# GarciaLnk/LlamaRec

Measured on AMD Instinct MI355X. Metric: users/sec through retrieve+rerank, higher is better.
Workload: dtype bf16; 1 GPU; beauty two-stage: LRURec(V=12086, L=50, D=64, 2 blocks) top-50 with history mask -> Llama-2-7b (32 layers, bf16, random init) single prefill -> verbalizer over 20 candidates; batching=token budget 32768 per step (llamarec_amd/packing.py), rmsnorm_folded_into_gemm=False, llama_layers=32, parallelism=dp1, collective_backend=nccl

## Files before the change

llamarec_amd/csrc/api_llama.hip:

```cpp
#include <math.h>
#include <stdlib.h>
#include <string.h>

#include <vector>

#include "llama_kernels.h"

typedef unsigned short u16;

extern "C" int lr_llama_create_ex(const LrLlamaConfig* cfg, const LrLlamaArch* arch, const LrLlamaWeightsDesc* w,
                                  lr_llama_t** out) {
  if (!cfg || !w || !out || !w->layers) LR_FAIL(LR_EINVAL, "lr_llama_create: null argument");
  const LrLlamaArch llama_arch = {0, 0, 1.0f, {0, 0, 0, 0, 0}};
  if (!arch) arch = &llama_arch;
  if (arch->norm_style < 0 || arch->norm_style > 1 || arch->mlp_act < 0 || arch->mlp_act > 1 ||
      !(arch->embed_scale > 0.f) || arch->embed_scale != arch->embed_scale)
    LR_FAIL(LR_EINVAL, "lr_llama_create_ex: arch norm_style=%d mlp_act=%d embed_scale=%g", arch->norm_style, arch->mlp_act,
            (double)arch->embed_scale);
  for (int i = 0; i < 5; ++i)
    if (arch->reserved[i]) LR_FAIL(LR_EINVAL, "lr_llama_create_ex: arch reserved word %d is not zero", i);
  if (cfg->num_layers < 1 || cfg->num_heads < 1 || cfg->num_kv_heads < 1 || cfg->vocab_size < 1)
    LR_FAIL(LR_EINVAL, "lr_llama_create: bad config");
  if (cfg->hidden_size % 8 != 0 || cfg->intermediate_size % 16 != 0)
    LR_FAIL(LR_EUNSUPPORTED, "lr_llama_create: hidden_size %% 8 and intermediate_size %% 16 must be 0");
// ... 9 lines not shown
      LR_FAIL(LR_EINVAL, "lr_llama_create: layer %d has a null weight", i);
  }
  lr_llama* h = (lr_llama*)calloc(1, sizeof(lr_llama));
  if (!h) LR_FAIL(LR_EINVAL, "lr_llama_create: out of host memory");
  h->cfg = *cfg;
  h->arch = *arch;
  h->embed = w->embed;
  h->final_norm = w->final_norm;
  h->lm_head = w->lm_head;
  h->prune_last = 1;
  h->layers = (LrLlamaLayerWeights*)malloc(sizeof(LrLlamaLayerWeights) * cfg->num_layers);
  memcpy(h->layers, w->layers, sizeof(LrLlamaLayerWeights) * cfg->num_layers);
  LR_CHECK_HIP(hipGetDevice(&h->device));
  *out = h;
  return LR_OK;
}

extern "C" int lr_llama_create(const LrLlamaConfig* cfg, const LrLlamaWeightsDesc* w, lr_llama_t** out) {
  return lr_llama_create_ex(cfg, nullptr, w, out);
}

extern "C" int lr_llama_set_variants(lr_llama_t* h, int32_t gemm_variant, int32_t attention_variant) {
  if (!h || (gemm_variant != 0 && gemm_variant != 1 && gemm_variant != 4 && gemm_variant != 5 && gemm_variant != 6) ||
      attention_variant < 0 || attention_variant > 9)
    LR_FAIL(LR_EINVAL, "lr_llama_set_variants: gemm in {0, 1, 4, 5, 6}, attention in {0, 1, 2, 3, 4, 5, 6, 7, 8, 9}");
  h->gemm_variant = gemm_variant;
  h->attn_variant = attention_variant;
  return LR_OK;
}

extern "C" int lr_llama_set_rope_scaling(lr_llama_t* h, const LrRopeScaling* s) {
  if (!h) LR_FAIL(LR_EINVAL, "lr_llama_set_rope_scaling: null handle");
  LR_RUN(lr_check_rope_scaling(s, "lr_llama_set_rope_scaling"));
  if (s) h->rope_scaling = *s;
  else memset(&h->rope_scaling, 0, sizeof(h->rope_scaling));
  return LR_OK;
}

static bool finite_nonneg(float v) { return v >= 0.f && v < __builtin_inff(); }

extern "C" int lr_llama_set_gemma2(lr_llama_t* h, const LrGemma2Ext* e) {
  if (!h) LR_FAIL(LR_EINVAL, "lr_llama_set_gemma2: null handle");
  const int L = h->cfg.num_layers;
  const uint16_t **an = nullptr, **mn = nullptr;
  float scale = 0.f;
  if (e) {
    if (!finite_nonneg(e->attn_softcap) || !finite_nonneg(e->final_softcap) || !finite_nonneg(e->attn_scale))
      LR_FAIL(LR_EINVAL, "lr_llama_set_gemma2: attn_softcap=%g final_softcap=%g attn_scale=%g (finite and >= 0)",
// ... 629 lines not shown
  return lr_launch_rope_table(cs, max_positions, head_dim, theta, (hipStream_t)hip_stream,
                              reinterpret_cast<unsigned*>(cs + (size_t)max_positions * head_dim), s);
}

extern "C" int lr_attention_varlen(const uint16_t* qkv, uint16_t* out, const int32_t* cu_seqlens,
                                   const int32_t* cu_seqlens_host, int32_t B, int32_t num_heads,
                                   int32_t num_kv_heads, int32_t head_dim, int32_t variant, void* hip_stream) {
  if (!qkv || !out || !cu_seqlens || !cu_seqlens_host || B < 1) LR_FAIL(LR_EINVAL, "lr_attention_varlen: bad argument");
  if (int rc = lr_check_segments(cu_seqlens_host, B, "lr_attention_varlen")) return rc;
  LrAttnKernel kernel;
  if (int rc = lr_resolve_attention({.variant = variant, .hd = head_dim}, &kernel)) return rc;
  return lr_launch_attention({.qkv = qkv, .out = out, .cu = cu_seqlens, .cu_host = cu_seqlens_host, .S = B,
                              .n_tok = cu_seqlens_host[B], .nh = num_heads, .nkv = num_kv_heads, .hd = head_dim},
                             kernel, (hipStream_t)hip_stream);
}

static int check_prefix_request(const char* who, const int32_t* cu_host, int S, int prefix_len, int nh, int nkv, int hd,
                                int variant) {
  if (!cu_host || S < 1 || prefix_len < 0 || nh < 1 || nkv < 1) LR_FAIL(LR_EINVAL, "%s: bad argument", who);
  if (int rc = lr_check_segments(cu_host, S, who)) return rc;
  if (nh % nkv != 0) LR_FAIL(LR_EINVAL, "%s: num_heads %d not a multiple of num_kv_heads %d", who, nh, nkv);
  if (prefix_len > 0 && (S < 2 || cu_host[1] != prefix_len))
    LR_FAIL(LR_EINVAL, "%s: segment 0 has %d rows, the shared prefix %d (and a prompt must follow it)", who, cu_host[1], prefix_len);
  const bool ok = (hd == 128 && (variant == 0 || variant == 2)) || (hd == 64 && (variant == 0 || variant == 5)) ||
                  (hd == 96 && (variant == 0 || variant == 7 || variant == 8)) || (hd == 256 && (variant == 0 || variant == 4 || variant == 9));
  if (!ok)
    LR_FAIL(LR_EUNSUPPORTED, "%s: variant %d at head_dim %d (0 / 2 at 128, 0 / 5 at 64, 0 / 7 / 8 at 96, 0 / 4 / 9 at 256)", who, variant, hd);
  return LR_OK;
}

extern "C" int lr_attention_varlen_prefix(const uint16_t* qkv, uint16_t* out, const int32_t* seg_starts,
                                          const int32_t* seg_starts_host, int32_t S, int32_t prefix_len, int32_t num_heads,
                                          int32_t num_kv_heads, int32_t head_dim, int32_t variant, void* hip_stream) {
  if (!qkv || !out || !seg_starts) LR_FAIL(LR_EINVAL, "lr_attention_varlen_prefix: null pointer");
  LR_RUN(check_prefix_request("lr_attention_varlen_prefix", seg_starts_host, S, prefix_len, num_heads, num_kv_heads, head_dim,
                              variant));
  LrAttnKernel kernel;
  LR_RUN(lr_resolve_attention({.variant = variant, .hd = head_dim, .prefix_len = prefix_len, .prefill = true}, &kernel));
  return lr_launch_attention({.qkv = qkv, .out = out, .cu = seg_starts, .cu_host = seg_starts_host, .S = S,
                              .n_tok = seg_starts_host[S], .nh = num_heads, .nkv = num_kv_heads, .hd = head_dim,
                              .prefix_len = prefix_len}, kernel, (hipStream_t)hip_stream);
}

extern "C" int lr_attention_last_rows(const uint16_t* kv, const uint16_t* q_last, uint16_t* out_last, const int32_t* seg_starts,
                                      const int32_t* seg_starts_host, int32_t S, int32_t prefix_len, int32_t num_heads,
                                      int32_t num_kv_heads, int32_t head_dim, int32_t variant, void* hip_stream) {
  if (!kv || !q_last || !out_last || !seg_starts) LR_FAIL(LR_EINVAL, "lr_attention_last_rows: null pointer");
  LR_RUN(check_prefix_request("lr_attention_last_rows", seg_starts_host, S, prefix_len, num_heads, num_kv_heads, head_dim,
                              variant));
  return lr_launch_attention_last(kv, q_last, out_last, seg_starts, seg_starts_host, S, seg_starts_host[S], num_heads,
// ... 456 lines not shown
```

llamarec_amd/csrc/api_llama_train.hip:

```cpp
#include <stdint.h>
#include <stdlib.h>
#include <string.h>

#include "llama_train.h"

typedef unsigned short u16;

struct lr_llama_lora {
  lr_llama* base;
  LrLoraTrainConfig cfg;
  LrLlamaLayerWeightsT* layers_t;
  const u16* lm_head_t;
  float *params, *grads, *m, *v;
  size_t n_params, per_layer;
  u16* work;
  size_t work_per_layer;
  float* scratch;
  int* ctr;
  uint32_t pass;
  int qcols, kcols, vcols;
  uint32_t mods;
  hipStream_t side;
  hipEvent_t ev_fork, ev_join;
  int deterministic;
// ... 519 lines not shown
  if (m < 1) LR_FAIL(LR_EINVAL, "lr_llama_lora_loss_grad: no labelled rows (m=%d)", m);
  hipStream_t st = (hipStream_t)hip_stream;
  const LrLlamaConfig& c = h->base->cfg;
  int n, maxT;
  LR_RUN(validate_batch(h, cu_seqlens_host, B, &n, &maxT));
  if (m > n) LR_FAIL(LR_EINVAL, "lr_llama_lora_loss_grad: %d labelled rows for %d tokens", m, n);
  const LoraMods md = lora_mods(c, h->cfg.r, h->mods);
  const bool det = h->deterministic != 0;
  const LoraWs ws = carve(c, md, n, B, m, c.num_layers, true, (char*)workspace, h->cfg.r, det, h->base->q_norm != nullptr);
  if (ws.total > workspace_bytes)
    LR_FAIL(LR_EWORKSPACE, "lr_llama_lora_loss_grad: workspace needs %zu bytes for %d tokens, have %zu", ws.total, n,
            workspace_bytes);
  const int d = c.hidden_size, f = c.intermediate_size, nh = c.num_heads, nkv = c.num_kv_heads, hd = c.head_dim;
  const int qw = (nh + 2 * nkv) * hd, r = h->cfg.r;
  const float scaling = h->cfg.alpha / (float)r, drop_p = h->cfg.dropout;
  const float drop_scale = drop_p > 0.f ? 1.0f / (1.0f - drop_p) : 1.0f;
  const int gv = h->base->gemm_variant == 5 ? 0 : h->base->gemm_variant;
  const int tw = md.tw, L = c.num_layers;
  LrAttnKernel fwd_kernel;
  LR_RUN(lr_resolve_attention({.variant = h->base->attn_variant, .hd = hd, .want_lse = true, .lora = true}, &fwd_kernel));
  const int attn_bwd_variant = fwd_kernel == LR_ATTN_HD64    ? 6
                               : fwd_kernel == LR_ATTN_HD96  ? 8
                               : fwd_kernel == LR_ATTN_HD256 ? 9
                                                             : h->base->attn_variant;
  h->pass += 1;
  if (!accumulate) LR_CHECK_HIP(hipMemsetAsync(h->grads, 0, h->n_params * sizeof(float), st));
  float* const scal = det ? ws.det_loss : h->scratch;
  float* const dp = ws.det_part;
  LR_CHECK_HIP(hipMemsetAsync(scal, 0, 2 * sizeof(float), st));
  LR_RUN(prep_adapters(h, st));
  LR_RUN(forward(h, packed_ids, cu_seqlens, cu_seqlens_host, B, n, maxT, ws, true, drop_p, st));

  LR_RUN(lr_launch_gather_rows(ws.x_final, loss_rows, m, d, ws.xg, st));
  LR_RUN(lr_launch_rmsnorm(ws.xg, h->base->final_norm, ws.hn, m, d, c.rms_eps, nullptr, st));
  LR_RUN(lr_launch_gemm({.A = ws.hn, .B = h->base->lm_head, .C = ws.logits, .M = m, .N = c.vocab_size, .K = d, .variant = gv}, st));
  LR_RUN(lr_launch_ce_bf16(ws.logits, m, c.vocab_size, loss_targets, grad_scale / (float)m, scal, st, det));
  LR_RUN(lr_launch_finish_loss(scal, m, out, st, det));
  LR_RUN(lr_launch_gemm({.A = ws.logits, .B = h->lm_head_t, .C = ws.dhn, .M = m, .N = d, .K = c.vocab_size, .variant = gv}, st));
  LR_CHECK_HIP(hipMemsetAsync(ws.dx, 0, (size_t)n * d * 2, st));
  LR_RUN(lr_launch_rmsnorm_bwd(ws.dhn, ws.xg, h->base->final_norm, nullptr, ws.dx, m, d, c.rms_eps, loss_rows, nullptr,
                               nullptr, 0, 0, 0.f, st));

  for (int l = c.num_layers - 1; l >= 0; --l) {
    const LrLlamaLayerWeights& w = h->base->layers[l];
    const LrLlamaLayerWeightsT& wt = h->layers_t[l];
    const LoraLayerSave s = slot(ws, l);
// ... 378 lines not shown
```

llamarec_amd/csrc/llama_attn.hip:

```cpp
#include <stdlib.h>

#include <type_traits>

#include "llama_kernels.h"
#include "lr_attn_util.h"
#include "lr_profile.h"

typedef unsigned short u16;
typedef __bf16 bf16x8 __attribute__((ext_vector_type(8)));
typedef __bf16 bf16x4 __attribute__((ext_vector_type(4)));
typedef short short4v __attribute__((ext_vector_type(4)));
typedef float floatx4 __attribute__((ext_vector_type(4)));
typedef u16 u16x4 __attribute__((ext_vector_type(4)));
typedef u16 u16x8 __attribute__((ext_vector_type(8)));

__global__ __launch_bounds__(256) void attn_generic_kernel(const u16* qkv, u16* out, const int32_t* cu, int B,
                                                           int n_tok, int nh, int nkv, int hd,
                                                           const int32_t* q_rows, float* lse, float scale_arg, float cap,
                                                           int window) {
  __shared__ float qs[4][256];
  const int wave = threadIdx.x >> 6, lane = threadIdx.x & 63;
  const int item = blockIdx.x * 4 + wave;
  if (item >= n_tok * nh) return;
  const int orow = item / nh, h = item % nh;
// ... 72 lines not shown
__device__ unsigned long long g_attn_stamps[64 * 8];
#define FA_WG_TRACE 8192
#ifdef LR_EXPERIMENTS
__device__ unsigned long long g_attn_wg[FA_WG_TRACE * 8];
#else
__device__ unsigned long long g_attn_wg[8];
#endif
#define FA_RT(dst)                                                                \
  if (STAMP) {                                                                    \
    __builtin_amdgcn_sched_barrier(0);                                            \
    asm volatile("s_memrealtime %0\n\ts_waitcnt lgkmcnt(0)" : "=s"(dst)::"memory"); \
    __builtin_amdgcn_sched_barrier(0);                                            \
  }
#define FA_STAMP(slot)                                                         \
  if (STAMP) {                                                                 \
    unsigned long long t_;                                                     \
    __builtin_amdgcn_sched_barrier(0);                                         \
    asm volatile("s_memtime %0\n\ts_waitcnt lgkmcnt(0)" : "=s"(t_)::"memory"); \
    __builtin_amdgcn_sched_barrier(0);                                         \
    stamp_acc[(slot)] += t_ - t_prev;                                          \
    t_prev = t_;                                                               \
  }

template <bool STAMP, bool LASTQ = false>
__global__ __launch_bounds__(256, 2) void attn_mfma128_kernel(const u16* __restrict__ qkv, u16* out,
                                                              const int32_t* cu, int prefix_len, int nh, int nkv,
                                                              int max_qblocks, int n_pairs, float* lse,
                                                              const u16* __restrict__ q_rows_last = nullptr) {
  unsigned long long stamp_acc[8] = {0, 0, 0, 0, 0, 0, 0, 0}, t_prev = 0;
  unsigned long long rt_entry = 0, rt_pro = 0, rt_loop = 0, rt_exit = 0;
  FA_RT(rt_entry)
  if (STAMP) asm volatile("s_memtime %0\n\ts_waitcnt lgkmcnt(0)" : "=s"(t_prev)::"memory");
  extern __shared__ __attribute__((aligned(16))) char smem[];
  const int hd = 128;
  int seg, h, qb;
  if (LASTQ) {
    const int id = blockIdx.x, stream = id & 7, pl = id >> 3;
    const int pair = pl * 8 + stream;
    if (pair >= n_pairs) return;
    seg = __builtin_amdgcn_readfirstlane(pair / nh);
    h = __builtin_amdgcn_readfirstlane(pair - seg * nh);
    if (prefix_len > 0 && seg == 0) return;
    qb = 0;
  } else {
    const int id = blockIdx.x, stream = id & 7, j = id >> 3;
    const int ppx = (n_pairs + 7) >> 3;
    const int n_light = min(max_qblocks, 2), n_heavy = max_qblocks - n_light;
    int pl;
    if (j < ppx * n_heavy) {
      pl = j / n_heavy;
      qb = max_qblocks - 1 - j % n_heavy;
// ... 8 lines not shown
    h = __builtin_amdgcn_readfirstlane(pair - seg * nh);
    qb = __builtin_amdgcn_readfirstlane(qb);
  }
  const int tok0 = cu[seg];
  const int P = (prefix_len > 0 && seg > 0) ? prefix_len : 0;
  const int T = P + cu[seg + 1] - tok0;
  if (LASTQ) qb = (T - 1) / FA_QROWS;
  if (qb * FA_QROWS >= T || (qb + 1) * FA_QROWS <= P) return;
  const int tid = threadIdx.x, lane = tid & 63;
  const int wave = __builtin_amdgcn_readfirstlane(tid >> 6);
  const int quad = lane >> 4, li = lane & 15;
  const int kvh = __builtin_amdgcn_readfirstlane(h / (nh / nkv));
  const int stride = LASTQ ? 2 * nkv * hd : (nh + 2 * nkv) * hd;
  const int koff0 = LASTQ ? kvh * hd : (nh + kvh) * hd, voff0 = koff0 + nkv * hd;
  const int vtok0 = tok0 - P;
  const u16* kbase = qkv + (size_t)vtok0 * stride + koff0;
  const u16* vbase = qkv + (size_t)vtok0 * stride + voff0;
  const u16* pkbase = qkv + koff0;
  const u16* pvbase = qkv + voff0;
  const int prompt = prefix_len > 0 ? seg - 1 : seg;

  bf16x8 qf[2][4];
  int qabs[2];
#pragma unroll
  for (int qt = 0; qt < 2; ++qt) {
    qabs[qt] = LASTQ ? T - 1 : qb * FA_QROWS + wave * 32 + qt * 16 + li;
    const int qr = min(max(qabs[qt], P), T - 1);
    const u16* qp = LASTQ ? q_rows_last + (size_t)prompt * nh * hd + h * hd + quad * 8
                          : qkv + (size_t)(vtok0 + qr) * stride + h * hd + quad * 8;
#pragma unroll
    for (int ks = 0; ks < 4; ++ks) qf[qt][ks] = *reinterpret_cast<const bf16x8*>(qp + ks * 32);
  }

  floatx4 ot[2][8];
#pragma unroll
  for (int qt = 0; qt < 2; ++qt)
#pragma unroll
    for (int dt = 0; dt < 8; ++dt) ot[qt][dt] = floatx4{0.f, 0.f, 0.f, 0.f};
  float m_run[2] = {-__builtin_inff(), -__builtin_inff()};
  float mthr[2] = {-__builtin_inff(), -__builtin_inff()};
  floatx4 l_acc[2] = {floatx4{0.f, 0.f, 0.f, 0.f}, floatx4{0.f, 0.f, 0.f, 0.f}};
  bf16x8 ones_f;
#pragma unroll
  for (int i = 0; i < 8; ++i) ones_f[i] = (__bf16)1.0f;

  const int q_last = min(qb * FA_QROWS + FA_QROWS - 1, T - 1);
  const int kb_last = q_last / FA_KB;
  const int wave_q_last = LASTQ ? T - 1 : qb * FA_QROWS + wave * 32 + 31;
  const float sl2 = 0.08838834764831845f * 1.4426950408889634f;
// ... 35 lines not shown
  };

  typedef __attribute__((address_space(3))) char lds_char;
  lds_char* const lds = (lds_char*)smem;
  lds_char *kb_off[4], *vb_off[8];
#pragma unroll
  for (int ks = 0; ks < 4; ++ks) kb_off[ks] = lds + (li * 256 + (((ks * 4 + quad) ^ li) << 4));
  {
    const int qp = li >> 2, p4 = li & 3;
#pragma unroll
    for (int dt = 0; dt < 8; ++dt) vb_off[dt] = lds + (v_off(quad * 4 + qp, dt * 2 + (p4 >> 1)) + 8 * (p4 & 1));
  }

  stage(0, 0);
#pragma unroll
  for (int qt = 0; qt < 2; ++qt)
#pragma unroll
    for (int ks = 0; ks < 4; ++ks) asm volatile("" ::"v"(qf[qt][ks]));
  asm volatile("s_waitcnt vmcnt(0)" ::: "memory");
  __syncthreads();
  FA_STAMP(0)
  FA_RT(rt_pro)

  auto block = [&](const int kb, auto buf_c) {
    constexpr int BUF = decltype(buf_c)::value;
    constexpr int KS = BUF * FA_STAGE_BYTES, VS = KS + FA_TILE_BYTES;
    if (kb < kb_last) stage(kb + 1, BUF ^ 1);
    FA_STAMP(1)

    if (kb * FA_KB <= wave_q_last && wave_q_last >= P && (!LASTQ || wave == 0)) {
      floatx4 st[2][4];
#pragma unroll
      for (int qt = 0; qt < 2; ++qt)
#pragma unroll
        for (int nt = 0; nt < 4; ++nt) st[qt][nt] = floatx4{0.f, 0.f, 0.f, 0.f};
      typedef __attribute__((address_space(3))) const bf16x8 lds_bf16x8;
      bf16x8 kf[2][4];
#pragma unroll
      for (int nt = 0; nt < 4; ++nt) kf[0][nt] = *reinterpret_cast<lds_bf16x8*>(kb_off[0] + (KS + nt * 4096));
#pragma unroll
      for (int ks = 0; ks < 4; ++ks) {
        if (ks < 3) {
#pragma unroll
          for (int nt = 0; nt < 4; ++nt)
            kf[(ks + 1) & 1][nt] = *reinterpret_cast<lds_bf16x8*>(kb_off[ks + 1] + (KS + nt * 4096));
        }
#pragma unroll
        for (int nt = 0; nt < 4; ++nt)
#pragma unroll
          for (int qt = 0; qt < 2; ++qt)
            st[qt][nt] = __builtin_amdgcn_mfma_f32_16x16x32_bf16(kf[ks & 1][nt], qf[qt][ks], st[qt][nt], 0, 0, 0);
      }

      if (STAMP) asm volatile("" ::"v"(st[0][0]), "v"(st[1][3]));
      FA_STAMP(2)
      bf16x8 pa[2][2];
      const bool diag = (kb * FA_KB + FA_KB - 1) > (LASTQ ? T - 1 : qb * FA_QROWS + wave * 32);
#pragma unroll
      for (int qt = 0; qt < 2; ++qt) {
        float mx = -__builtin_inff();
        if (diag) {
#pragma unroll
          for (int nt = 0; nt < 4; ++nt)
#pragma unroll
            for (int r = 0; r < 4; ++r) {
              const int key = kb * FA_KB + nt * 16 + quad * 4 + r;
              st[qt][nt][r] = (key <= qabs[qt]) ? st[qt][nt][r] : -__builtin_inff();
            }
          __builtin_amdgcn_sched_barrier(0);
        }
        mx = fa_max3(st[qt][0][0], st[qt][0][1], st[qt][0][2]);
        mx = fa_max3(mx, st[qt][0][3], st[qt][1][0]);
#pragma unroll
        for (int nt = 1; nt < 4; ++nt) {
          mx = fa_max3(mx, st[qt][nt][1], st[qt][nt][2]);
          if (nt < 3) mx = fa_max3(mx, st[qt][nt][3], st[qt][nt + 1][0]);
        }
        mx = fa_max2(mx, st[qt][3][3]);
        if (__any(mx > mthr[qt])) {
          const float rmx = fa_max_xor16_32(mx);
          const bool grew = rmx > mthr[qt];
          const float m_new = grew ? rmx * sl2 : m_run[qt];
          const float alpha = __builtin_amdgcn_exp2f(m_run[qt] - m_new);
#pragma unroll
          for (int r = 0; r < 4; ++r) l_acc[qt][r] *= alpha;
#pragma unroll
          for (int dt = 0; dt < 8; ++dt)
#pragma unroll
            for (int r = 0; r < 4; ++r) ot[qt][dt][r] *= alpha;
          m_run[qt] = m_new;
          mthr[qt] = (m_new + FA_DEFER) * inv_sl2;
        }
        const float m_new = m_run[qt];
#pragma unroll
        for (int nt = 0; nt < 4; ++nt)
#pragma unroll
          for (int r = 0; r < 4; ++r) {
            const float p = __builtin_amdgcn_exp2f(__builtin_fmaf(st[qt][nt][r], sl2, -m_new));
            pa[qt][nt >> 1][(nt & 1) * 4 + r] = (__bf16)p;
          }
      }

      if (STAMP) asm volatile("" ::"v"(pa[0][0]), "v"(pa[1][1]));
      FA_STAMP(3)
#pragma unroll
      for (int ks2 = 0; ks2 < 2; ++ks2) {
#pragma unroll
        for (int qt = 0; qt < 2; ++qt) l_acc[qt] = __builtin_amdgcn_mfma_f32_16x16x32_bf16(ones_f, pa[qt][ks2], l_acc[qt], 0, 0, 0);
#pragma unroll
        for (int dt = 0; dt < 8; ++dt) {
          const short4v t0 = __builtin_amdgcn_ds_read_tr16_b64_v4i16(
              (__attribute__((address_space(3))) short4v*)(vb_off[dt] + (VS + ks2 * 8192)));
          const short4v t1 = __builtin_amdgcn_ds_read_tr16_b64_v4i16(
              (__attribute__((address_space(3))) short4v*)(vb_off[dt] + (VS + ks2 * 8192 + 4096)));
          bf16x8 vf;
          const bf16x4 b0 = __builtin_bit_cast(bf16x4, t0), b1 = __builtin_bit_cast(bf16x4, t1);
#pragma unroll
          for (int r = 0; r < 4; ++r) {
            vf[r] = b0[r];
            vf[4 + r] = b1[r];
          }
#pragma unroll
          for (int qt = 0; qt < 2; ++qt)
            ot[qt][dt] = __builtin_amdgcn_mfma_f32_16x16x32_bf16(vf, pa[qt][ks2], ot[qt][dt], 0, 0, 0);
        }
      }
    }
    if (STAMP) asm volatile("" ::"v"(ot[0][0]), "v"(ot[1][7]));
    FA_STAMP(4)
    asm volatile("s_waitcnt vmcnt(0)" ::: "memory");
    __syncthreads();
    FA_STAMP(5)
  };
  for (int kb = 0; kb <= kb_last; kb += 2) {
    block(kb, std::integral_constant<int, 0>{});
    if (kb + 1 <= kb_last) block(kb + 1, std::integral_constant<int, 1>{});
  }

  FA_RT(rt_loop)
#pragma unroll
  for (int qt = 0; qt < 2; ++qt) {
    const float l = l_acc[qt][0];
    const float inv = 1.0f / l;
    if (!LASTQ && qabs[qt] < T && qabs[qt] >= P && lse && quad == 0)
      lse[(size_t)(vtok0 + qabs[qt]) * nh + h] = (m_run[qt] + __builtin_amdgcn_logf(l)) * 0.6931471805599453f;
    const bool live = LASTQ ? (wave == 0 && qt == 0 && li == 0) : (qabs[qt] < T && qabs[qt] >= P);
    u16* op = out + (size_t)(LASTQ ? prompt : vtok0 + (live ? qabs[qt] : P)) * nh * hd + h * hd + (quad & 1) * 16 + (quad >> 1) * 8;
#pragma unroll
    for (int k = 0; k < 4; ++k) {
      unsigned a[2], b[2];
#pragma unroll
      for (int w = 0; w < 2; ++w) {
        a[w] = (unsigned)f2bf(ot[qt][2 * k][2 * w] * inv) | ((unsigned)f2bf(ot[qt][2 * k][2 * w + 1] * inv) << 16);
        b[w] = (unsigned)f2bf(ot[qt][2 * k + 1][2 * w] * inv) | ((unsigned)f2bf(ot[qt][2 * k + 1][2 * w + 1] * inv) << 16);
        const auto sw = __builtin_amdgcn_permlane16_swap(a[w], b[w], false, false);
        a[w] = sw[0];
        b[w] = sw[1];
      }
      if (live) {
// ... 32 lines not shown
extern "C" int lr_debug_attn_stamps(unsigned long long* out, int n) {
  if (!out || n < 1 || n > 64 * 8) LR_FAIL(LR_EINVAL, "lr_debug_attn_stamps: bad arguments");
  LR_CHECK_HIP(hipMemcpyFromSymbol(out, HIP_SYMBOL(g_attn_stamps), (size_t)n * sizeof(unsigned long long)));
  return LR_OK;
}
#endif

int lr_launch_attention_rows(const u16* qkv, u16* out, const int32_t* cu, int B, const int32_t* q_rows,
                             int n_rows, int nh, int nkv, int hd, hipStream_t st, float scale, float cap, int window) {
  if (n_rows <= 0) return LR_OK;
  if (window < 0) LR_FAIL(LR_EINVAL, "attention: window %d", window);
  if (hd > 256) LR_FAIL(LR_EUNSUPPORTED, "attention: head_dim %d > 256", hd);
  const int items = n_rows * nh;
  hipLaunchKernelGGL(attn_generic_kernel, dim3((items + 3) / 4), dim3(256), 0, st, qkv, out, cu, B, n_rows,
                     nh, nkv, hd, q_rows, (float*)nullptr, scale, cap, window);
  LR_CHECK_LAUNCH("attn_generic_kernel(rows)");
  return LR_OK;
}

int lr_resolve_attention(const LrAttnRequest& r, LrAttnKernel* kernel) {
  const int hd = r.hd;
  if (r.cap > 0.f) {
    if (r.want_lse) LR_FAIL(LR_EINVAL, "attention: no lse with a soft cap");
    if (r.variant == 2 || r.variant == 3 || r.variant == 5 || r.variant == 6 || ((r.variant == 7 || r.variant == 8) && hd == 96) ||
        (r.variant == 9 && hd == 256))
      LR_FAIL(LR_EUNSUPPORTED, "attention variant %d has no soft-capped form (0 / 4 at head_dim 256, 1 generic)", r.variant);
    if (r.variant != 0 && r.variant != 1 && r.variant != 4) LR_FAIL(LR_EINVAL, "attention: unknown variant %d", r.variant);
    if (r.variant != 1 && hd == 256 && r.cap <= LR_SOFTCAP_MFMA_MAX) {
      *kernel = LR_ATTN_HD256;
      return LR_OK;
    }
    if (r.prefix_len > 0) LR_FAIL(LR_EUNSUPPORTED, "attention: the generic kernel reads no shared prefix (soft cap, head_dim %d)", hd);
    *kernel = LR_ATTN_GENERIC;
    return LR_OK;
  }
  switch (r.variant) {
    case 0:
      if (hd == 128) *kernel = (r.have_items_ws && !r.prefill) ? LR_ATTN_ROWS256 : LR_ATTN_MFMA128;
      else if (hd == 256 && (r.prefill || r.lora || r.prefix_len > 0)) *kernel = LR_ATTN_HD256;
      else if (hd == 96 && (r.prefill || r.lora || r.prefix_len > 0)) *kernel = LR_ATTN_HD96;
      else *kernel = (hd == 64 && (r.prefill || r.lora || r.prefix_len > 0)) ? LR_ATTN_HD64 : LR_ATTN_GENERIC;
      if (r.prefix_len > 0 && *kernel == LR_ATTN_GENERIC)
        LR_FAIL(LR_EUNSUPPORTED, "attention: no kernel reads a shared prefix at head_dim %d", hd);
      if (r.prefix_len > 0 && r.want_lse && hd != 128)
        LR_FAIL(LR_EINVAL, "attention: no lse with a shared prefix at head_dim %d", hd);
      return LR_OK;
    case 1:
// ... 18 lines not shown
      if (hd != 64) LR_FAIL(LR_EUNSUPPORTED, "attention variant 5 needs head_dim 64 (got %d)", hd);
      *kernel = LR_ATTN_HD64;
      return LR_OK;
    case 6:
      if (hd != 64) LR_FAIL(LR_EUNSUPPORTED, "attention variant 6 needs head_dim 64 (got %d)", hd);
      if (r.want_lse && r.prefix_len > 0) LR_FAIL(LR_EINVAL, "attention variant 6 writes no lse with a shared prefix");
      *kernel = LR_ATTN_HD64;
      return LR_OK;
    case 7:
      if (r.want_lse) LR_FAIL(LR_EINVAL, "attention variant 7 (head_dim-96 MFMA) writes no lse");
      if (hd != 96) LR_FAIL(LR_EUNSUPPORTED, "attention variant 7 needs head_dim 96 (got %d)", hd);
      *kernel = LR_ATTN_HD96;
      return LR_OK;
    case 8:
      if (hd != 96) LR_FAIL(LR_EUNSUPPORTED, "attention variant 8 needs head_dim 96 (got %d)", hd);
      if (r.want_lse && r.prefix_len > 0) LR_FAIL(LR_EINVAL, "attention variant 8 writes no lse with a shared prefix");
      *kernel = LR_ATTN_HD96;
      return LR_OK;
    case 9:
      if (hd != 256) LR_FAIL(LR_EUNSUPPORTED, "attention variant 9 needs head_dim 256 (got %d)", hd);
      if (r.want_lse && r.prefix_len > 0) LR_FAIL(LR_EINVAL, "attention variant 9 writes no lse with a shared prefix");
      *kernel = LR_ATTN_HD256;
      return LR_OK;
  }
  LR_FAIL(LR_EINVAL, "attention: unknown variant %d (0 auto, 1 generic, 2 = head_dim-128 MFMA, 3 = 256-row tiles, "
          "4 = head_dim-256 MFMA, 5 = head_dim-64 MFMA, 6 = head_dim-64 MFMA for training, 7 = head_dim-96 MFMA, "
          "8 = head_dim-96 MFMA for training, 9 = head_dim-256 MFMA for training)", r.variant);
}

int lr_launch_attention(const LrAttnArgs& a, LrAttnKernel kernel, hipStream_t st) {
  const int32_t* cu_host = a.cu_host;
  const int B = a.S, n_tok = a.n_tok, nh = a.nh, nkv = a.nkv, hd = a.hd, prefix_len = a.prefix_len;
  if (n_tok <= 0 || B <= 0) return LR_OK;
  if (a.cap < 0.f || a.scale < 0.f || a.cap != a.cap || a.scale != a.scale)
    LR_FAIL(LR_EINVAL, "attention: scale %g cap %g", (double)a.scale, (double)a.cap);
  if (a.cap > 0.f && kernel != LR_ATTN_HD256 && kernel != LR_ATTN_GENERIC)
    LR_FAIL(LR_EUNSUPPORTED, "attention: kernel %d has no soft-capped form", (int)kernel);
  if (a.window < 0) LR_FAIL(LR_EINVAL, "attention: window %d", a.window);
  if (a.window > 0 && ((kernel != LR_ATTN_HD256 && kernel != LR_ATTN_GENERIC) || prefix_len != 0 || a.lse || a.cap > 0.f))
    LR_FAIL(LR_EUNSUPPORTED, "attention: a sliding window runs on the head_dim-256 MFMA kernel or the generic one, without a "
            "shared prefix, lse or a soft cap (kernel %d, prefix %d)", (int)kernel, prefix_len);
  if (kernel == LR_ATTN_ROWS256) return lr_launch_attention256(a, st);
  if (nh % nkv != 0) LR_FAIL(LR_EINVAL, "attention: num_heads %d not a multiple of num_kv_heads %d", nh, nkv);
  if (kernel == LR_ATTN_HD256) {
    if (prefix_len < 0 || (a.lse && (prefix_len > 0 || a.cap > 0.f)))
      LR_FAIL(LR_EINVAL, "attention: the head_dim-256 MFMA kernel writes no lse with a shared prefix or a soft cap (prefix %d)",
              prefix_len);
    if (a.cap > 0.f) return lr_launch_attention_hd256_softcap(a, st);
    if (a.window > 0) return lr_launch_attention_hd256_window(a, st);
    return prefix_len > 0 ? lr_launch_attention_hd256_prefix(a, st) : lr_launch_attention_hd256(a, st);
  }
  if (kernel == LR_ATTN_HD64) {
    if (prefix_len < 0) LR_FAIL(LR_EINVAL, "attention: shared prefix of %d tokens", prefix_len);
    return prefix_len > 0 ? lr_launch_attention_hd64_prefix(a, st) : lr_launch_attention_hd64(a, st);
  }
  if (kernel == LR_ATTN_HD96) {
    if (prefix_len < 0 || (prefix_len > 0 && a.lse))
      LR_FAIL(LR_EINVAL, "attention: the head_dim-96 MFMA kernel writes no lse with a shared prefix (prefix %d)", prefix_len);
    return prefix_len > 0 ? lr_launch_attention_hd96_prefix(a, st) : lr_launch_attention_hd96(a, st);
  }
  if (prefix_len < 0 || (prefix_len > 0 && (kernel != LR_ATTN_MFMA128 || cu_host[1] - cu_host[0] != prefix_len)))
    LR_FAIL(LR_EINVAL, "attention: shared prefix of %d tokens needs the head_dim-128 MFMA kernel and segment 0 = the prefix",
            prefix_len);
  const LrAttnPlan pl = lr_attn_plan(cu_host, B, prefix_len, nh, hd, FA_QROWS, nh);
  LrProfScope prof(kernel == LR_ATTN_MFMA128 ? LR_PROF_ATTN_MFMA : LR_PROF_ATTN_GENERIC, pl.work, st);
  if (kernel == LR_ATTN_MFMA128) {
    if (hd != 128) LR_FAIL(LR_EUNSUPPORTED, "attention variant 2 needs head_dim 128 (got %d)", hd);
    const int mq = pl.mq;
    if (mq == 0) return LR_OK;
    LR_RUN(lr_attn_check_grid(pl));
    if ((long long)n_tok * (nh + 2 * nkv) * hd * 2 > 0x7fffffffLL * 2)
      LR_FAIL(LR_EUNSUPPORTED, "attention: packed qkv of %d tokens exceeds the 4 GiB a buffer descriptor addresses", n_tok);
    const int n_pairs = (int)pl.n_pairs;
    const unsigned grid = (unsigned)pl.grid;
    static bool lds_set[LR_MAX_DEVICES] = {};
    if (int rc = lr_ensure_dynamic_lds(reinterpret_cast<const void*>(attn_mfma128_kernel<false>), 2 * FA_STAGE_BYTES, lds_set))
      return rc;
#ifdef LR_EXPERIMENTS
    static bool lds_set_stamp[LR_MAX_DEVICES] = {};
    const char* stamp_env = getenv("LR_ATTN_STAMPS");
    if (stamp_env && stamp_env[0] == '1') {
      const char* one_env = getenv("LR_ATTN_ONE_PER_CU");
      const int lds_bytes = (one_env && one_env[0] == '1') ? 104 * 1024 : 2 * FA_STAGE_BYTES;
      if (int rc = lr_ensure_dynamic_lds(reinterpret_cast<const void*>(attn_mfma128_kernel<true>), 104 * 1024, lds_set_stamp))
        return rc;
      hipLaunchKernelGGL(attn_mfma128_kernel<true>, dim3(grid), dim3(256), lds_bytes, st, a.qkv, a.out, a.cu,
                         prefix_len, nh, nkv, mq, n_pairs, a.lse);
    } else
#endif
      hipLaunchKernelGGL(attn_mfma128_kernel<false>, dim3(grid), dim3(256), 2 * FA_STAGE_BYTES, st, a.qkv, a.out, a.cu,
                         prefix_len, nh, nkv, mq, n_pairs, a.lse);
    LR_CHECK_LAUNCH("attn_mfma128_kernel");
  } else {
    if (hd > 256) LR_FAIL(LR_EUNSUPPORTED, "attention: head_dim %d > 256", hd);
    const int items = n_tok * nh;
    hipLaunchKernelGGL(attn_generic_kernel, dim3((items + 3) / 4), dim3(256), 0, st, a.qkv, a.out, a.cu, B,
                       n_tok, nh, nkv, hd, (const int32_t*)nullptr, a.lse, a.scale, a.cap, a.window);
// ... 41 lines not shown
```

llamarec_amd/csrc/llama_kernels.h:

```cpp
#ifndef LLAMA_KERNELS_H
#define LLAMA_KERNELS_H

#include "lr_common.h"
#include "lr_profile.h"

__device__ __forceinline__ float bf2f(unsigned short b) {
  return __builtin_bit_cast(float, (unsigned int)b << 16);
}
__device__ __forceinline__ unsigned short f2bf(float f) {
  return __builtin_bit_cast(unsigned short, (__bf16)f);
}
__device__ __forceinline__ unsigned short swiglu_bf16(float g, float u) {
  float s = bf2f(f2bf(g * __builtin_amdgcn_rcpf(1.0f + __expf(-g))));
  return f2bf(s * u);
}

__device__ __forceinline__ unsigned short geglu_bf16(float g, float u) {
  const float t = tanhf(0.7978845608028654f * (g + 0.044715f * g * g * g));
  float s = bf2f(f2bf(0.5f * g * (1.0f + t)));
  return f2bf(s * u);
}
template <int NS>
__device__ __forceinline__ unsigned short rms_apply(unsigned short w, unsigned short x, float rstd) {
  if (NS == 0) return f2bf(bf2f(w) * bf2f(f2bf(bf2f(x) * rstd)));
// ... 113 lines not shown
    const double P = (prefix_len > 0 && b > 0) ? prefix_len : 0, T = P + cu_host[b + 1] - cu_host[b];
    p.work += 4.0 * nh * hd * (T * (T + 1) / 2 - P * (P + 1) / 2);
    p.maxT = p.maxT > (int)T ? p.maxT : (int)T;
  }
  p.mq = (p.maxT + q_rows - 1) / q_rows;
  p.n_pairs = (long long)S * pairs_per_prompt;
  p.grid = 8 * ((p.n_pairs + 7) / 8) * p.mq;
  return p;
}
static inline LrAttnPlan lr_attn_plan_last(const int32_t* cu_host, int S, int prefix_len, int nh, int hd, int grid_multiple) {
  LrAttnPlan p;
  for (int b = (prefix_len > 0 ? 1 : 0); b < S; ++b)
    p.work += 4.0 * nh * hd * (double)((prefix_len > 0 ? prefix_len : 0) + cu_host[b + 1] - cu_host[b]);
  p.n_pairs = (long long)S * nh;
  p.grid = grid_multiple * ((p.n_pairs + grid_multiple - 1) / grid_multiple);
  return p;
}
static inline int lr_attn_check_grid(const LrAttnPlan& p) {
  if (p.grid > 0x7fffffffLL) LR_FAIL(LR_EUNSUPPORTED, "attention: %lld workgroups exceed the grid limit", p.grid);
  return LR_OK;
}

enum LrAttnKernel {
  LR_ATTN_GENERIC = 1, LR_ATTN_MFMA128 = 2, LR_ATTN_ROWS256 = 3, LR_ATTN_HD256 = 4, LR_ATTN_HD64 = 5, LR_ATTN_HD96 = 7
};

#define LR_SOFTCAP_MFMA_MAX 256.0f
static inline bool lr_attention_reads_prefix(int variant, int hd, float cap = 0.f) {
  if (cap > 0.f) return hd == 256 && (variant == 0 || variant == 4) && cap <= LR_SOFTCAP_MFMA_MAX;
  if (hd == 128) return variant != 1;
  if (hd == 64) return variant == 0 || variant == 5 || variant == 6;
  if (hd == 96) return variant == 0 || variant == 7 || variant == 8;
  if (hd == 256) return variant == 0 || variant == 4 || variant == 9;
  return false;
}
static inline bool lr_attention_has_last_row_mode(int kernel, int hd) {
  return (hd == 128 && kernel != 1 ) || kernel == 4  || kernel == 5  ||
         kernel == 7 ;
}
struct LrAttnRequest {
  int variant, hd, prefix_len = 0;
  bool want_lse = false, have_items_ws = false, prefill = false, lora = false;
  float cap = 0.f;
};
int lr_resolve_attention(const LrAttnRequest& r, LrAttnKernel* kernel);

struct LrAttnArgs {
// ... 112 lines not shown
```

Baseline: 159.2 users/s.

## Balance causal attention waves with mirrored row groups and per-group diagonal skipping

The default head_dim-128 MFMA attention kernel now gives each wave a mirrored pair of 16-row query groups (wave and 7-wave) instead of 32 contiguous rows. It runs full key blocks on a fast unmasked path and handles diagonal blocks per group, skipping MFMA tiles that lie fully above the causal diagonal. This is meant to even out causal work across waves and cut wasted score and PV compute on diagonal tiles. The old contiguous mapping stays reachable as a new variant 10. The cost is more code paths, extra register pressure and more branching.

```diff
diff --git a/llamarec_amd/csrc/api_llama.hip b/llamarec_amd/csrc/api_llama.hip
--- a/llamarec_amd/csrc/api_llama.hip
+++ b/llamarec_amd/csrc/api_llama.hip
@@ -55,8 +55,8 @@
 
 extern "C" int lr_llama_set_variants(lr_llama_t* h, int32_t gemm_variant, int32_t attention_variant) {
   if (!h || (gemm_variant != 0 && gemm_variant != 1 && gemm_variant != 4 && gemm_variant != 5 && gemm_variant != 6) ||
-      attention_variant < 0 || attention_variant > 9)
-    LR_FAIL(LR_EINVAL, "lr_llama_set_variants: gemm in {0, 1, 4, 5, 6}, attention in {0, 1, 2, 3, 4, 5, 6, 7, 8, 9}");
+      attention_variant < 0 || attention_variant > 10)
+    LR_FAIL(LR_EINVAL, "lr_llama_set_variants: gemm in {0, 1, 4, 5, 6}, attention in {0, 1, 2, 3, 4, 5, 6, 7, 8, 9, 10}");
   h->gemm_variant = gemm_variant;
   h->attn_variant = attention_variant;
   return LR_OK;
@@ -732,10 +732,10 @@
   if (nh % nkv != 0) LR_FAIL(LR_EINVAL, "%s: num_heads %d not a multiple of num_kv_heads %d", who, nh, nkv);
   if (prefix_len > 0 && (S < 2 || cu_host[1] != prefix_len))
     LR_FAIL(LR_EINVAL, "%s: segment 0 has %d rows, the shared prefix %d (and a prompt must follow it)", who, cu_host[1], prefix_len);
-  const bool ok = (hd == 128 && (variant == 0 || variant == 2)) || (hd == 64 && (variant == 0 || variant == 5)) ||
+  const bool ok = (hd == 128 && (variant == 0 || variant == 2 || variant == 10)) || (hd == 64 && (variant == 0 || variant == 5)) ||
                   (hd == 96 && (variant == 0 || variant == 7 || variant == 8)) || (hd == 256 && (variant == 0 || variant == 4 || variant == 9));
   if (!ok)
-    LR_FAIL(LR_EUNSUPPORTED, "%s: variant %d at head_dim %d (0 / 2 at 128, 0 / 5 at 64, 0 / 7 / 8 at 96, 0 / 4 / 9 at 256)", who, variant, hd);
+    LR_FAIL(LR_EUNSUPPORTED, "%s: variant %d at head_dim %d (0 / 2 / 10 at 128, 0 / 5 at 64, 0 / 7 / 8 at 96, 0 / 4 / 9 at 256)", who, variant, hd);
   return LR_OK;
 }
 
diff --git a/llamarec_amd/csrc/api_llama_train.hip b/llamarec_amd/csrc/api_llama_train.hip
--- a/llamarec_amd/csrc/api_llama_train.hip
+++ b/llamarec_amd/csrc/api_llama_train.hip
@@ -565,6 +565,7 @@
   const int attn_bwd_variant = fwd_kernel == LR_ATTN_HD64    ? 6
                                : fwd_kernel == LR_ATTN_HD96  ? 8
                                : fwd_kernel == LR_ATTN_HD256 ? 9
+                               : fwd_kernel == LR_ATTN_MFMA128_STRAIGHT ? 2
                                                              : h->base->attn_variant;
   h->pass += 1;
   if (!accumulate) LR_CHECK_HIP(hipMemsetAsync(h->grads, 0, h->n_params * sizeof(float), st));
diff --git a/llamarec_amd/csrc/llama_attn.hip b/llamarec_amd/csrc/llama_attn.hip
--- a/llamarec_amd/csrc/llama_attn.hip
+++ b/llamarec_amd/csrc/llama_attn.hip
@@ -118,11 +118,12 @@
     t_prev = t_;                                                               \
   }
 
-template <bool STAMP, bool LASTQ = false>
+template <bool STAMP, bool LASTQ = false, bool STRAIGHT = false>
 __global__ __launch_bounds__(256, 2) void attn_mfma128_kernel(const u16* __restrict__ qkv, u16* out,
                                                               const int32_t* cu, int prefix_len, int nh, int nkv,
                                                               int max_qblocks, int n_pairs, float* lse,
                                                               const u16* __restrict__ q_rows_last = nullptr) {
+  constexpr bool GROUPS = !LASTQ && !STRAIGHT;
   unsigned long long stamp_acc[8] = {0, 0, 0, 0, 0, 0, 0, 0}, t_prev = 0;
   unsigned long long rt_entry = 0, rt_pro = 0, rt_loop = 0, rt_exit = 0;
   FA_RT(rt_entry)
@@ -177,9 +178,15 @@
 
   bf16x8 qf[2][4];
   int qabs[2];
+  int g_need[2] = {-1, -1}, g_nv[2] = {4, 4};
 #pragma unroll
   for (int qt = 0; qt < 2; ++qt) {
-    qabs[qt] = LASTQ ? T - 1 : qb * FA_QROWS + wave * 32 + qt * 16 + li;
+    const int g0 = qb * FA_QROWS + (GROUPS ? (qt ? 7 - wave : wave) * 16 : wave * 32 + qt * 16);
+    if (GROUPS && g0 < T && g0 + 15 >= P) {
+      g_need[qt] = g0 / FA_KB;
+      g_nv[qt] = ((g0 & (FA_KB - 1)) >> 4) + 1;
+    }
+    qabs[qt] = LASTQ ? T - 1 : g0 + li;
     const int qr = min(max(qabs[qt], P), T - 1);
     const u16* qp = LASTQ ? q_rows_last + (size_t)prompt * nh * hd + h * hd + quad * 8
                           : qkv + (size_t)(vtok0 + qr) * stride + h * hd + quad * 8;
@@ -261,19 +268,24 @@
   FA_STAMP(0)
   FA_RT(rt_pro)
 
-  auto block = [&](const int kb, auto buf_c) {
+  auto block = [&](const int kb, auto buf_c, auto hot_c) {
     constexpr int BUF = decltype(buf_c)::value;
+    constexpr bool HOT = decltype(hot_c)::value;
     constexpr int KS = BUF * FA_STAGE_BYTES, VS = KS + FA_TILE_BYTES;
     if (kb < kb_last) stage(kb + 1, BUF ^ 1);
     FA_STAMP(1)
 
-    if (kb * FA_KB <= wave_q_last && wave_q_last >= P && (!LASTQ || wave == 0)) {
-      floatx4 st[2][4];
+    typedef __attribute__((address_space(3))) const bf16x8 lds_bf16x8;
+    typedef std::integral_constant<int, 0> c0;
+    typedef std::integral_constant<int, 1> c1;
+    typedef std::integral_constant<int, 3> c3;
+    typedef std::integral_constant<int, 4> c4;
+
+    auto scores_pair = [&](floatx4(&st)[2][4]) __attribute__((always_inline)) {
 #pragma unroll
       for (int qt = 0; qt < 2; ++qt)
 #pragma unroll
         for (int nt = 0; nt < 4; ++nt) st[qt][nt] = floatx4{0.f, 0.f, 0.f, 0.f};
-      typedef __attribute__((address_space(3))) const bf16x8 lds_bf16x8;
       bf16x8 kf[2][4];
 #pragma unroll
       for (int nt = 0; nt < 4; ++nt) kf[0][nt] = *reinterpret_cast<lds_bf16x8*>(kb_off[0] + (KS + nt * 4096));
@@ -290,80 +302,141 @@
           for (int qt = 0; qt < 2; ++qt)
             st[qt][nt] = __builtin_amdgcn_mfma_f32_16x16x32_bf16(kf[ks & 1][nt], qf[qt][ks], st[qt][nt], 0, 0, 0);
       }
-
-      if (STAMP) asm volatile("" ::"v"(st[0][0]), "v"(st[1][3]));
-      FA_STAMP(2)
-      bf16x8 pa[2][2];
-      const bool diag = (kb * FA_KB + FA_KB - 1) > (LASTQ ? T - 1 : qb * FA_QROWS + wave * 32);
-#pragma unroll
-      for (int qt = 0; qt < 2; ++qt) {
-        float mx = -__builtin_inff();
-        if (diag) {
-#pragma unroll
-          for (int nt = 0; nt < 4; ++nt)
-#pragma unroll
-            for (int r = 0; r < 4; ++r) {
-              const int key = kb * FA_KB + nt * 16 + quad * 4 + r;
-              st[qt][nt][r] = (key <= qabs[qt]) ? st[qt][nt][r] : -__builtin_inff();
-            }
-          __builtin_amdgcn_sched_barrier(0);
-        }
-        mx = fa_max3(st[qt][0][0], st[qt][0][1], st[qt][0][2]);
-        mx = fa_max3(mx, st[qt][0][3], st[qt][1][0]);
-#pragma unroll
-        for (int nt = 1; nt < 4; ++nt) {
-          mx = fa_max3(mx, st[qt][nt][1], st[qt][nt][2]);
-          if (nt < 3) mx = fa_max3(mx, st[qt][nt][3], st[qt][nt + 1][0]);
-        }
-        mx = fa_max2(mx, st[qt][3][3]);
-        if (__any(mx > mthr[qt])) {
-          const float rmx = fa_max_xor16_32(mx);
-          const bool grew = rmx > mthr[qt];
-          const float m_new = grew ? rmx * sl2 : m_run[qt];
-          const float alpha = __builtin_amdgcn_exp2f(m_run[qt] - m_new);
-#pragma unroll
-          for (int r = 0; r < 4; ++r) l_acc[qt][r] *= alpha;
-#pragma unroll
-          for (int dt = 0; dt < 8; ++dt)
-#pragma unroll
-            for (int r = 0; r < 4; ++r) ot[qt][dt][r] *= alpha;
-          m_run[qt] = m_new;
-          mthr[qt] = (m_new + FA_DEFER) * inv_sl2;
-        }
-        const float m_new = m_run[qt];
+    };
+
+    auto softmax_group = [&](auto qt_c, floatx4(&st)[2][4], bf16x8(&pa)[2][2], const bool masked, auto nv_c) __attribute__((always_inline)) {
+      constexpr int qt = decltype(qt_c)::value;
+      constexpr bool NV_RT = std::is_same<decltype(nv_c), int>::value;
+      const int nv = nv_c;
+      float mx;
+      if (masked) {
 #pragma unroll
         for (int nt = 0; nt < 4; ++nt)
+#pragma unroll
+          for (int r = 0; r < 4; ++r) {
+            const int key = kb * FA_KB + nt * 16 + quad * 4 + r;
+            st[qt][nt][r] = (key <= qabs[qt]) ? st[qt][nt][r] : -__builtin_inff();
+          }
+        __builtin_amdgcn_sched_barrier(0);
+      }
+      mx = fa_max3(st[qt][0][0], st[qt][0][1], st[qt][0][2]);
+      mx = fa_max3(mx, st[qt][0][3], st[qt][1][0]);
+#pragma unroll
+      for (int nt = 1; nt < 4; ++nt) {
+        mx = fa_max3(mx, st[qt][nt][1], st[qt][nt][2]);
+        if (nt < 3) mx = fa_max3(mx, st[qt][nt][3], st[qt][nt + 1][0]);
+      }
+      mx = fa_max2(mx, st[qt][3][3]);
+      if (__any(mx > mthr[qt])) {
+        const float rmx = fa_max_xor16_32(mx);
+        const bool grew = rmx > mthr[qt];
+        const float m_new = grew ? rmx * sl2 : m_run[qt];
+        const float alpha = __builtin_amdgcn_exp2f(m_run[qt] - m_new);
+#pragma unroll
+        for (int r = 0; r < 4; ++r) l_acc[qt][r] *= alpha;
+#pragma unroll
+        for (int dt = 0; dt < 8; ++dt)
+#pragma unroll
+          for (int r = 0; r < 4; ++r) ot[qt][dt][r] *= alpha;
+        m_run[qt] = m_new;
+        mthr[qt] = (m_new + FA_DEFER) * inv_sl2;
+      }
+      const float m_new = m_run[qt];
+#pragma unroll
+      for (int nt = 0; nt < 4; ++nt) {
+        if (nt < nv) {
+          if constexpr (NV_RT) asm volatile("");
 #pragma unroll
           for (int r = 0; r < 4; ++r) {
             const float p = __builtin_amdgcn_exp2f(__builtin_fmaf(st[qt][nt][r], sl2, -m_new));
             pa[qt][nt >> 1][(nt & 1) * 4 + r] = (__bf16)p;
           }
-      }
-
+        } else {
+#pragma unroll
+          for (int r = 0; r < 4; ++r) pa[qt][nt >> 1][(nt & 1) * 4 + r] = (__bf16)0.0f;
+        }
+      }
+    };
+
+    auto pv_step = [&](auto qm_c, auto ks2_c, bf16x8(&pa)[2][2]) __attribute__((always_inline)) {
+      constexpr int QM = decltype(qm_c)::value, ks2 = decltype(ks2_c)::value;
+#pragma unroll
+      for (int qt = 0; qt < 2; ++qt)
+        if ((QM >> qt) & 1) l_acc[qt] = __builtin_amdgcn_mfma_f32_16x16x32_bf16(ones_f, pa[qt][ks2], l_acc[qt], 0, 0, 0);
+#pragma unroll
+      for (int dt = 0; dt < 8; ++dt) {
+        const short4v t0 = __builtin_amdgcn_ds_read_tr16_b64_v4i16(
+            (__attribute__((address_space(3))) short4v*)(vb_off[dt] + (VS + ks2 * 8192)));
+        const short4v t1 = __builtin_amdgcn_ds_read_tr16_b64_v4i16(
+            (__attribute__((address_space(3))) short4v*)(vb_off[dt] + (VS + ks2 * 8192 + 4096)));
+        bf16x8 vf;
+        const bf16x4 b0 = __builtin_bit_cast(bf16x4, t0), b1 = __builtin_bit_cast(bf16x4, t1);
+#pragma unroll
+        for (int r = 0; r < 4; ++r) {
+          vf[r] = b0[r];
+          vf[4 + r] = b1[r];
+        }
+#pragma unroll
+        for (int qt = 0; qt < 2; ++qt)
+          if ((QM >> qt) & 1) ot[qt][dt] = __builtin_amdgcn_mfma_f32_16x16x32_bf16(vf, pa[qt][ks2], ot[qt][dt], 0, 0, 0);
+      }
+    };
+
+    auto both_groups = [&](const bool masked) __attribute__((always_inline)) {
+      floatx4 st[2][4];
+      bf16x8 pa[2][2];
+      scores_pair(st);
+      __builtin_amdgcn_sched_barrier(0);
+      if (STAMP) asm volatile("" ::"v"(st[0][0]), "v"(st[1][3]));
+      FA_STAMP(2)
+      softmax_group(c0{}, st, pa, masked, c4{});
+      softmax_group(c1{}, st, pa, masked, c4{});
       if (STAMP) asm volatile("" ::"v"(pa[0][0]), "v"(pa[1][1]));
       FA_STAMP(3)
-#pragma unroll
-      for (int ks2 = 0; ks2 < 2; ++ks2) {
-#pragma unroll
-        for (int qt = 0; qt < 2; ++qt) l_acc[qt] = __builtin_amdgcn_mfma_f32_16x16x32_bf16(ones_f, pa[qt][ks2], l_acc[qt], 0, 0, 0);
-#pragma unroll
-        for (int dt = 0; dt < 8; ++dt) {
-          const short4v t0 = __builtin_amdgcn_ds_read_tr16_b64_v4i16(
-              (__attribute__((address_space(3))) short4v*)(vb_off[dt] + (VS + ks2 * 8192)));
-          const short4v t1 = __builtin_amdgcn_ds_read_tr16_b64_v4i16(
-              (__attribute__((address_space(3))) short4v*)(vb_off[dt] + (VS + ks2 * 8192 + 4096)));
-          bf16x8 vf;
-          const bf16x4 b0 = __builtin_bit_cast(bf16x4, t0), b1 = __builtin_bit_cast(bf16x4, t1);
-#pragma unroll
-          for (int r = 0; r < 4; ++r) {
-            vf[r] = b0[r];
-            vf[4 + r] = b1[r];
+      pv_step(c3{}, c0{}, pa);
+      pv_step(c3{}, c1{}, pa);
+    };
+    auto one_group = [&](auto qt_c, const int nv, const bool diag) __attribute__((always_inline)) {
+      constexpr int qt = decltype(qt_c)::value;
+      floatx4 st[2][4];
+      bf16x8 pa[2][2];
+      bf16x8 kf[2][4];
+#pragma unroll
+      for (int ks = 0; ks < 4; ++ks) kf[0][ks] = *reinterpret_cast<lds_bf16x8*>(kb_off[ks] + KS);
+#pragma unroll
+      for (int nt = 0; nt < 4; ++nt) {
+        if (nt < nv) {
+          if (nt < 3) {
+#pragma unroll
+            for (int ks = 0; ks < 4; ++ks) kf[(nt + 1) & 1][ks] = *reinterpret_cast<lds_bf16x8*>(kb_off[ks] + (KS + (nt + 1) * 4096));
           }
-#pragma unroll
-          for (int qt = 0; qt < 2; ++qt)
-            ot[qt][dt] = __builtin_amdgcn_mfma_f32_16x16x32_bf16(vf, pa[qt][ks2], ot[qt][dt], 0, 0, 0);
+          floatx4 acc = floatx4{0.f, 0.f, 0.f, 0.f};
+#pragma unroll
+          for (int ks = 0; ks < 4; ++ks) acc = __builtin_amdgcn_mfma_f32_16x16x32_bf16(kf[nt & 1][ks], qf[qt][ks], acc, 0, 0, 0);
+          if (diag && nt == nv - 1) {
+#pragma unroll
+            for (int r = 0; r < 4; ++r) acc[r] = (quad * 4 + r <= li) ? acc[r] : -__builtin_inff();
+          }
+          st[qt][nt] = acc;
+        } else {
+          st[qt][nt] = floatx4{-__builtin_inff(), -__builtin_inff(), -__builtin_inff(), -__builtin_inff()};
         }
       }
+      softmax_group(qt_c, st, pa, false, nv);
+      pv_step(std::integral_constant<int, 1 << qt>{}, c0{}, pa);
+      if (nv > 2) pv_step(std::integral_constant<int, 1 << qt>{}, c1{}, pa);
+    };
+
+    if constexpr (GROUPS) {
+      const int d0 = g_need[0] - kb, d1 = g_need[1] - kb;
+      if (HOT) {
+        both_groups(false);
+      } else {
+        if (d0 >= 0) one_group(c0{}, d0 == 0 ? g_nv[0] : 4, d0 == 0);
+        if (d1 >= 0) one_group(c1{}, d1 == 0 ? g_nv[1] : 4, d1 == 0);
+      }
+    } else if (kb * FA_KB <= wave_q_last && wave_q_last >= P && (!LASTQ || wave == 0)) {
+      both_groups((kb * FA_KB + FA_KB - 1) > (LASTQ ? T - 1 : qb * FA_QROWS + wave * 32));
     }
     if (STAMP) asm volatile("" ::"v"(ot[0][0]), "v"(ot[1][7]));
     FA_STAMP(4)
@@ -371,9 +444,17 @@
     __syncthreads();
     FA_STAMP(5)
   };
-  for (int kb = 0; kb <= kb_last; kb += 2) {
-    block(kb, std::integral_constant<int, 0>{});
-    if (kb + 1 <= kb_last) block(kb + 1, std::integral_constant<int, 1>{});
+  int kb = 0;
+  if constexpr (GROUPS) {
+    if (g_need[0] >= 0 && g_need[1] >= 0)
+      for (; kb < 2 * qb; kb += 2) {
+        block(kb, std::integral_constant<int, 0>{}, std::true_type{});
+        block(kb + 1, std::integral_constant<int, 1>{}, std::true_type{});
+      }
+  }
+  for (; kb <= kb_last; kb += 2) {
+    block(kb, std::integral_constant<int, 0>{}, std::false_type{});
+    if (kb + 1 <= kb_last) block(kb + 1, std::integral_constant<int, 1>{}, std::false_type{});
   }
 
   FA_RT(rt_loop)
@@ -452,7 +533,7 @@
   const int hd = r.hd;
   if (r.cap > 0.f) {
     if (r.want_lse) LR_FAIL(LR_EINVAL, "attention: no lse with a soft cap");
-    if (r.variant == 2 || r.variant == 3 || r.variant == 5 || r.variant == 6 || ((r.variant == 7 || r.variant == 8) && hd == 96) ||
+    if (r.variant == 2 || r.variant == 3 || r.variant == 5 || r.variant == 6 || r.variant == 10 || ((r.variant == 7 || r.variant == 8) && hd == 96) ||
         (r.variant == 9 && hd == 256))
       LR_FAIL(LR_EUNSUPPORTED, "attention variant %d has no soft-capped form (0 / 4 at head_dim 256, 1 generic)", r.variant);
     if (r.variant != 0 && r.variant != 1 && r.variant != 4) LR_FAIL(LR_EINVAL, "attention: unknown variant %d", r.variant);
@@ -517,10 +598,14 @@
       if (r.want_lse && r.prefix_len > 0) LR_FAIL(LR_EINVAL, "attention variant 9 writes no lse with a shared prefix");
       *kernel = LR_ATTN_HD256;
       return LR_OK;
+    case 10:
+      *kernel = LR_ATTN_MFMA128_STRAIGHT;
+      return LR_OK;
   }
   LR_FAIL(LR_EINVAL, "attention: unknown variant %d (0 auto, 1 generic, 2 = head_dim-128 MFMA, 3 = 256-row tiles, "
           "4 = head_dim-256 MFMA, 5 = head_dim-64 MFMA, 6 = head_dim-64 MFMA for training, 7 = head_dim-96 MFMA, "
-          "8 = head_dim-96 MFMA for training, 9 = head_dim-256 MFMA for training)", r.variant);
+          "8 = head_dim-96 MFMA for training, 9 = head_dim-256 MFMA for training, 10 = head_dim-128 MFMA, straight row "
+          "mapping)", r.variant);
 }
 
 int lr_launch_attention(const LrAttnArgs& a, LrAttnKernel kernel, hipStream_t st) {
@@ -554,13 +639,14 @@
       LR_FAIL(LR_EINVAL, "attention: the head_dim-96 MFMA kernel writes no lse with a shared prefix (prefix %d)", prefix_len);
     return prefix_len > 0 ? lr_launch_attention_hd96_prefix(a, st) : lr_launch_attention_hd96(a, st);
   }
-  if (prefix_len < 0 || (prefix_len > 0 && (kernel != LR_ATTN_MFMA128 || cu_host[1] - cu_host[0] != prefix_len)))
+  const bool mfma128 = kernel == LR_ATTN_MFMA128 || kernel == LR_ATTN_MFMA128_STRAIGHT;
+  if (prefix_len < 0 || (prefix_len > 0 && (!mfma128 || cu_host[1] - cu_host[0] != prefix_len)))
     LR_FAIL(LR_EINVAL, "attention: shared prefix of %d tokens needs the head_dim-128 MFMA kernel and segment 0 = the prefix",
             prefix_len);
   const LrAttnPlan pl = lr_attn_plan(cu_host, B, prefix_len, nh, hd, FA_QROWS, nh);
-  LrProfScope prof(kernel == LR_ATTN_MFMA128 ? LR_PROF_ATTN_MFMA : LR_PROF_ATTN_GENERIC, pl.work, st);
-  if (kernel == LR_ATTN_MFMA128) {
-    if (hd != 128) LR_FAIL(LR_EUNSUPPORTED, "attention variant 2 needs head_dim 128 (got %d)", hd);
+  LrProfScope prof(mfma128 ? LR_PROF_ATTN_MFMA : LR_PROF_ATTN_GENERIC, pl.work, st);
+  if (mfma128) {
+    if (hd != 128) LR_FAIL(LR_EUNSUPPORTED, "attention variant %d needs head_dim 128 (got %d)", (int)kernel, hd);
     const int mq = pl.mq;
     if (mq == 0) return LR_OK;
     LR_RUN(lr_attn_check_grid(pl));
@@ -568,6 +654,16 @@
       LR_FAIL(LR_EUNSUPPORTED, "attention: packed qkv of %d tokens exceeds the 4 GiB a buffer descriptor addresses", n_tok);
     const int n_pairs = (int)pl.n_pairs;
     const unsigned grid = (unsigned)pl.grid;
+    if (kernel == LR_ATTN_MFMA128_STRAIGHT) {
+      static bool lds_set_straight[LR_MAX_DEVICES] = {};
+      if (int rc = lr_ensure_dynamic_lds(reinterpret_cast<const void*>(attn_mfma128_kernel<false, false, true>), 2 * FA_STAGE_BYTES,
+                                         lds_set_straight))
+        return rc;
+      hipLaunchKernelGGL((attn_mfma128_kernel<false, false, true>), dim3(grid), dim3(256), 2 * FA_STAGE_BYTES, st, a.qkv, a.out, a.cu,
+                         prefix_len, nh, nkv, mq, n_pairs, a.lse);
+      LR_CHECK_LAUNCH("attn_mfma128_kernel<straight>");
+      return LR_OK;
+    }
     static bool lds_set[LR_MAX_DEVICES] = {};
     if (int rc = lr_ensure_dynamic_lds(reinterpret_cast<const void*>(attn_mfma128_kernel<false>), 2 * FA_STAGE_BYTES, lds_set))
       return rc;
diff --git a/llamarec_amd/csrc/llama_kernels.h b/llamarec_amd/csrc/llama_kernels.h
--- a/llamarec_amd/csrc/llama_kernels.h
+++ b/llamarec_amd/csrc/llama_kernels.h
@@ -159,7 +159,8 @@
 }
 
 enum LrAttnKernel {
-  LR_ATTN_GENERIC = 1, LR_ATTN_MFMA128 = 2, LR_ATTN_ROWS256 = 3, LR_ATTN_HD256 = 4, LR_ATTN_HD64 = 5, LR_ATTN_HD96 = 7
+  LR_ATTN_GENERIC = 1, LR_ATTN_MFMA128 = 2, LR_ATTN_ROWS256 = 3, LR_ATTN_HD256 = 4, LR_ATTN_HD64 = 5, LR_ATTN_HD96 = 7,
+  LR_ATTN_MFMA128_STRAIGHT = 10
 };
 
 #define LR_SOFTCAP_MFMA_MAX 256.0f
```

Result: no change. 159.5 users/s, median of 6 (+0.2%).
